# michelebanfi/qLDPC

Measured on AMD Instinct MI355X. Metric: syndromes/sec at 50 BP iters, [[288,12,18]] code, higher is better.
Workload: dtype f64; 1 GPU; BASELINE.json configs[3]: [[288,12,18]] BB code, sum-product BP, max_iter 50, every syndrome runs all 50 iterations (mode M2); max_iter=50, threads_per_block=1024, grid=512, lds_bytes=124000

## Files before the change

### qldpc_amd/csrc/qbp_kernels.hpp

```cpp
#pragma once

#include <hip/hip_runtime.h>
#include <stdint.h>

#include <type_traits>

#include "qbp_check.hpp"
#include "qbp_mc.hpp"

#ifndef QBP_WIDE_JG
#define QBP_WIDE_JG 4
#endif
#ifndef QBP_WIDE_HOLD_R
#define QBP_WIDE_HOLD_R 1
#endif
#ifndef QBP_WIDE_PACK
#define QBP_WIDE_PACK 0
#endif
#ifndef QBP_SMALL_HOLD_R
#define QBP_SMALL_HOLD_R 1
#endif
#ifndef QBP_SMALL_PACK
#define QBP_SMALL_PACK 0
#endif
#ifndef QBP_MC_HOLD_R
#define QBP_MC_HOLD_R 0
#endif
#ifndef QBP_MC_PACK
#define QBP_MC_PACK 0
#endif
#ifndef QBP_WORK_CHUNK_SMALL_CODES
#define QBP_WORK_CHUNK_SMALL_CODES 1
#endif
#ifndef QBP_WORK_CHUNK_FIXED
#define QBP_WORK_CHUNK_FIXED 0
#endif

namespace qbp {

constexpr int FUSED_R2_OFF_BYTES = 57344;

struct FusedParams {
    const uint8_t* syndromes;
    const double* prior;
    long long B;
    int m, n;
    int S;
    int slot_stride;
    int max_iter;
    unsigned flags;
    int padded;
    int n_words4;
    int r0_table;
    double alpha, damping, clip_llr;
    uint8_t* hard;
    uint8_t* converged;
    int32_t* iters;
    double* llr;
    const int32_t* tab_var;
    const uint16_t* tab_nbr;
    const uint32_t* tab_writer;
    const int32_t* iso_vars;
    int n_iso;
    unsigned long long* work_counter;
    const unsigned long long* lx_cols;
    long long trial_begin;
    unsigned long long seed;
    unsigned threshold;
    int draws;
    int half_distance;
    long long* counters;
    const uint8_t* errors_in;
    long long* fail_list;
    unsigned long long* fail_count;
    uint8_t* fail_syn;
    double* fail_llr;
    uint8_t* fail_hard;
    uint8_t* fail_err;
    const uint32_t* thr_cols;
    int n_budgets;
    int budgets[MAX_BUDGETS];
};

typedef const FusedParams __attribute__((address_space(4)))* ColdArgs;
__device__ __forceinline__ ColdArgs cold_args()
{
    ColdArgs p = (ColdArgs)__builtin_amdgcn_kernarg_segment_ptr();
    asm volatile("" : "+s"(p));
    return p;
}
#define COLD(field) (cold_args()->field)

__device__ __forceinline__ int work_chunk_for(int avg4)
{
    return avg4 < 12 ? 8 : avg4 < 28 ? 4 : avg4 < 60 ? 2 : 1;
}

__device__ __forceinline__ void mc_classify(unsigned long long* mc_lmask, int* mc_weight,
                                            int* mc_diff, int* cnt, int slot, int conv, int it,
                                            int half_distance, bool deferred)
{
    if (deferred) {
        cnt[0] += 1; cnt[6] += 1; cnt[7] += it;
        return;
    }
    const unsigned long long lm = mc_lmask[slot];
    const int ew = mc_weight[slot];
    const int df = mc_diff[slot];
    mc_lmask[slot] = 0ull; mc_weight[slot] = 0; mc_diff[slot] = 0;
    mc_count_trial(cnt, lm, ew, df, conv, it, half_distance);
}

template <int DC, int DV, int VARIANT, bool MC, bool FORCE_FULL, int MAX_THREADS, int MIN_WAVES_PER_SIMD,
          bool ONE_BARRIER = false>
__global__ __launch_bounds__(MAX_THREADS, MIN_WAVES_PER_SIMD) void bp_fused_kernel(const FusedParams P)
{
    constexpr bool ONE_BAR = ONE_BARRIER && FORCE_FULL && !MC;
    constexpr bool BUDGETS = MC && QBP_MC_BUDGETS != 0;
    extern __shared__ __attribute__((aligned(16))) double smem_all[];
    constexpr NpT np_tab = 0u;
    double* const smem = smem_all + NP_LDS_DOUBLES;
    const int tid = threadIdx.x;
    const int m = P.m;
    const int S = P.S;
    const int slot = tid / m;
    const int c = tid - slot * m;
    const bool lane_valid = slot < S;
    const bool leader = lane_valid && c == 0;
    const int sl = lane_valid ? slot : 0;

    double* const Rs = smem + (size_t)sl * P.slot_stride;
    const int zoff = DC * m;
    double* const pri_lds = smem + (ONE_BAR ? FUSED_R2_OFF_BYTES / 8 : 0) + (size_t)S * P.slot_stride;
    const bool use_r0 = !FORCE_FULL && P.r0_table != 0;
    double* const r0_lds = pri_lds + DC * m;
    long long* const next_work = reinterpret_cast<long long*>(r0_lds + (use_r0 ? 2 * DC * m : 0));
    long long* const chunk_ends = next_work + S;
    unsigned long long* const mc_lmask = reinterpret_cast<unsigned long long*>(chunk_ends + S);
    int* const words = reinterpret_cast<int*>(mc_lmask + S);
    int* const flag0 = words;
    int* const mc_weight = words + 3 * S;
    int* const mc_diff = words + 4 * S;
    int* const work_avg = words + 5 * S;
    int* const active_count = words + 6 * S;
    int slot_counters = NUM_COUNTERS;
    if constexpr (BUDGETS) slot_counters = 2 * COLD(n_budgets) * NUM_COUNTERS;
    int* const mc_count = words + 6 * S + 1 + sl * slot_counters;
    int* const var_lds = words + 6 * S + 1 + S * slot_counters;
    unsigned err_par = 0;
    auto err_buf = [&]() -> unsigned char* {
        const int n4 = COLD(n_words4) * 4;
        return reinterpret_cast<unsigned char*>(var_lds + DC * m) + (size_t)(sl + (err_par ? S : 0)) * n4;
    };

    auto check_step = [&](const double (&q)[DC], unsigned sb, auto&& put) {
        check_row<VARIANT, DC, (DC > 6)>(q, sb, P.alpha, true, np_tab, put);
    };

    constexpr bool PACK_NBR = (DC > 6 && QBP_WIDE_PACK != 0) || (MC && QBP_MC_PACK != 0) ||
                              (DC <= 6 && !MC && QBP_SMALL_PACK != 0);
    constexpr int NBR_W = PACK_NBR ? (DV + 1) / 2 : DV;
    unsigned nbr[DC][NBR_W];
    unsigned wmask = 0;
    unsigned vmask = 0;
#pragma unroll
    for (int j = 0; j < DC; ++j) {
        const int v = lane_valid ? P.tab_var[j * m + c] : -1;
        vmask |= (v >= 0 ? 1u : 0u) << j;
        if (slot == 0) {
            pri_lds[j * m + c] = v >= 0 ? P.prior[v] : __builtin_inf();
            var_lds[j * m + c] = v;
        }
#pragma unroll
        for (int k = 0; k < DV; ++k)
        {
            const unsigned o = lane_valid ? P.tab_nbr[(j * DV + k) * m + c] : (unsigned)zoff;
            if constexpr (PACK_NBR) {
                if (k & 1) nbr[j][k / 2] |= o << 16; else nbr[j][k / 2] = o;
            } else {
                nbr[j][k] = o;
            }
        }
    }
    if (lane_valid) wmask = P.tab_writer[c];
    if (lds_address(smem_all) != np_tab) __builtin_trap();
    np_tables_to_lds(smem_all, tid, blockDim.x);
    if (use_r0) __syncthreads();
    if (use_r0 && lane_valid && slot == 0) {
        double qp[DC];
#pragma unroll
        for (int j = 0; j < DC; ++j) qp[j] = pri_lds[j * m + c];
        check_step(qp, 0u, [&](int j, double r) { r0_lds[j * m + c] = r; });
        check_step(qp, 1u, [&](int j, double r) { r0_lds[(DC + j) * m + c] = r; });
    }

    const long long B = P.B;
    const long long total_slots = (long long)gridDim.x * S;
    const double one_minus_damping = 1.0 - P.damping;
    const int max_iter = P.max_iter;

    auto work_chunk = [&](long long handed_out, int by_cost) -> int {
        if (QBP_WORK_CHUNK_FIXED) return FORCE_FULL ? 1 : 8;
        const long long rem = B - handed_out;
        const int share = rem >= 16 * total_slots ? 8 : rem >= 8 * total_slots ? 4 : rem >= 4 * total_slots ? 2 : 1;
        const int ch = share > by_cost ? share : by_cost;
        const int f = QBP_WORK_CHUNK_SMALL_CODES ? (m <= 36 ? 4 : m <= 72 ? 2 : 1) : 1;
        return (f > 1 && ch == 8 && rem >= (long long)16 * f * total_slots) ? 8 * f : ch;
    };
    long long b = lane_valid ? (long long)blockIdx.x * S + slot : B;
    bool active = b < B;

    if (leader) {
        Rs[zoff] = 0.0;
        if constexpr (ONE_BAR) Rs[FUSED_R2_OFF_BYTES / 8 + zoff] = 0.0;
        flag0[slot] = 0;
        flag0[S + slot] = 0;
        flag0[2 * S + slot] = 0;
        mc_lmask[slot] = 0ull;
        mc_weight[slot] = 0;
        mc_diff[slot] = 0;
        if (slot == 0) *work_avg = 4 * P.max_iter;
        if constexpr (BUDGETS) {
            for (int i = 0; i < slot_counters; ++i) mc_count[i] = 0;
        } else if constexpr (MC) {
            for (int i = 0; i < NUM_COUNTERS; ++i) mc_count[i] = 0;
        }
        const int ch = work_chunk(9 * total_slots, 1);
        const long long first =
            B > total_slots ? total_slots + (long long)atomicAdd(P.work_counter, (unsigned long long)ch) : B;
        next_work[slot] = first;
        chunk_ends[slot] = first + ch;
    }
    if (tid == 0) {
        long long first = (long long)blockIdx.x * S;
        long long cnt = B - first;
        *active_count = (int)(cnt < 0 ? 0 : (cnt > S ? S : cnt));
    }

    constexpr bool HOLD_R = MC ? (QBP_MC_HOLD_R != 0 && DC <= 6) : (DC <= 6 ? QBP_SMALL_HOLD_R != 0 : QBP_WIDE_HOLD_R != 0);

    double Q[DC];
    double R[HOLD_R ? DC : 1];
    unsigned sbit = 0, ebits = 0;
    int it = 0;
    bool frozen = false;
    int bj = 0, ck_it = 0;

    auto start_syndrome = [&]() {
        it = 0;
        frozen = false;
        if constexpr (BUDGETS) { bj = 0; ck_it = COLD(budgets)[0] - 1; }
#pragma unroll
        for (int j = 0; j < DC; ++j) Q[j] = pri_lds[j * m + c];
        if constexpr (MC) {
            ebits = 0;
            const unsigned char* const err_lds = err_buf();
#pragma unroll
            for (int j = 0; j < DC; ++j) {
                const int v = var_lds[j * m + c];
                if (v >= 0) ebits |= (unsigned)err_lds[v] << j;
            }
            sbit = __builtin_popcount(ebits) & 1u;
        } else {
            sbit = COLD(syndromes)[b * m + c] & 1u;
        }
    };
    bool need_start = active;
    __syncthreads();

    int refill = 0;
    bool mc_pending = false;
    int mc_pending_conv = 0, mc_pending_it = 0;
    int mc_pending_row = 0;
    auto pending_row = [&]() -> int* {
        if constexpr (BUDGETS)
            return mc_count + ((mc_pending_conv ? COLD(n_budgets) : 0) + mc_pending_row) * NUM_COUNTERS;
        else
            return mc_count;
    };

    double val_keep[DC];
    auto emit_decode = [&](const double (&val)[DC], bool conv, int it_out) {
        const ColdArgs ca = cold_args();
        double* const o_llr = ca->llr;
        uint8_t* const o_hard = ca->hard;
        const long long row = b * ca->n;
#pragma unroll
        for (int j = 0; j < DC; ++j) {
            if ((wmask >> j) & 1u) {
                const long long o = row + var_lds[j * m + c];
                if (o_llr) o_llr[o] = val[j];
                if (o_hard) o_hard[o] = (uint8_t)(val[j] < 0.0);
            }
        }
        const int n_iso = ca->n_iso;
        for (int i = c; i < n_iso; i += m) {
            const int v = COLD(iso_vars)[i];
            const double pv = COLD(prior)[v];
            if (o_llr) o_llr[row + v] = pv;
            if (o_hard) o_hard[row + v] = pv < 0.0;
        }
        if (c == 0) {
            if (ca->converged) ca->converged[b] = conv;
            if (ca->iters) ca->iters[b] = it_out;
        }
    };
    int f_cur = 0, f_next = 1, f_prev = 2;
    int wg_it = 0;

    auto phase_body = [&](auto par_tag) -> bool {
        constexpr int PAR = decltype(par_tag)::value;
        double* const Rw = ONE_BAR ? Rs + PAR * (FUSED_R2_OFF_BYTES / 8) : Rs;
        double val_phase[DC];
        double (&val)[DC] = ONE_BAR ? val_keep : val_phase;
        if constexpr (MC) {
            if (need_start) {
                err_par ^= 1u;
                unsigned* const err_words = reinterpret_cast<unsigned*>(err_buf());
                const unsigned long long trial = (unsigned long long)(COLD(trial_begin) + b);
#if QBP_MC_COLS
                const uint32_t* const thr = COLD(thr_cols);
                for (int g = c; g < P.n_words4; g += m)
                    err_words[g] = mc_error_quad_cols(trial, g, COLD(draws), COLD(seed), thr);
#else
                const uint8_t* const ein = COLD(errors_in);
                for (int g = c; g < P.n_words4; g += m)
                    err_words[g] = ein ? mc_stored_quad(ein + b * COLD(n), g, COLD(n))
                                       : mc_error_quad(trial, g, COLD(draws), COLD(seed), COLD(threshold));
#endif
            }
            __syncthreads();
        }
        if (need_start) { start_syndrome(); need_start = false; }
        if (active) {
            if (use_r0 && it == 0) {
                const double* const r0 = r0_lds + (sbit ? DC * m : 0);
#pragma unroll
                for (int j = 0; j < DC; ++j) {
                    const double r = r0[j * m + c];
                    Rw[j * m + c] = r;
                    if constexpr (HOLD_R) R[j] = r;
                }
            } else {
                check_step(Q, sbit, [&](int j, double r) {
                    Rw[j * m + c] = r;
                    if constexpr (HOLD_R) R[j] = r;
                });
            }
        }
        __syncthreads();
        if (*active_count == 0) return true;

        if constexpr (ONE_BAR) {
            if (active && it > 0 && !frozen && flag0[f_prev * S + slot] == 0) {
                emit_decode(val, true, it - 1);
                frozen = true;
            }
        }
        if (active) {
            bool odd = sbit != 0;
            constexpr int JG = (DC * DV <= 18) ? DC : QBP_WIDE_JG;
#pragma unroll
            for (int j0 = 0; j0 < DC; j0 += JG) {
                double rr[JG][DV];
                double rown[HOLD_R ? 1 : JG];
#pragma unroll
                for (int jj = 0; jj < JG; ++jj) {
#pragma unroll
                    for (int k = 0; k < DV; ++k)
                        if (j0 + jj < DC) {
                            if constexpr (PACK_NBR) {
                                unsigned o;
                                unsigned pk = nbr[j0 + jj][k / 2];
                                asm volatile("" : "+v"(pk));
                                o = (k & 1) ? pk >> 16 : pk & 0xffffu;
                                rr[jj][k] = Rw[o];
                            } else {
                                rr[jj][k] = Rw[nbr[j0 + jj][k]];
                            }
                        }
                    if constexpr (!HOLD_R)
                        if (j0 + jj < DC) rown[jj] = Rw[(j0 + jj) * m + c];
                }
                __builtin_amdgcn_sched_barrier(0);
#pragma unroll
                for (int jj = 0; jj < JG; ++jj) {
                    const int j = j0 + jj;
                    if (j >= DC) break;
                    double s = rr[jj][0];
#pragma unroll
                    for (int k = 1; k < DV; ++k) s = s + rr[jj][k];
                    val[j] = s + pri_lds[j * m + c];
                    odd ^= val[j] < 0.0;
                    double r_own;
                    if constexpr (HOLD_R) r_own = R[j]; else r_own = rown[jj];
                    const double qn = val[j] - r_own;
                    if constexpr (VARIANT == 0) {
                        Q[j] = qn;
                    } else {
                        Q[j] = damped_q(qn, Q[j], P.damping, one_minus_damping, P.clip_llr);
                    }
                }
            }
            if (P.padded) {
#pragma unroll
                for (int j = 0; j < DC; ++j)
                    if (!((vmask >> j) & 1u)) Q[j] = __builtin_inf();
            }
            if (odd) flag0[f_cur * S + slot] = 1;
        }
        if (leader) {
            flag0[f_next * S + slot] = 0;
            if (refill) {
                long long nx = next_work[slot] + 1;
                if (nx == chunk_ends[slot]) {
                    const int ch = work_chunk(nx, refill);
                    nx = total_slots +
                         (long long)atomicAdd(COLD(work_counter), (unsigned long long)ch);
                    chunk_ends[slot] = nx + ch;
                }
                next_work[slot] = nx;
                refill = 0;
            }
            if constexpr (MC) {
                if (mc_pending) {
                    mc_classify(mc_lmask, mc_weight, mc_diff, pending_row(), slot, mc_pending_conv,
                                mc_pending_it, COLD(half_distance),
                                COLD(fail_list) != nullptr && !mc_pending_conv);
                    mc_pending = false;
                }
            }
        }
        const bool settle = !ONE_BAR || wg_it == max_iter - 1;
        if (settle) __syncthreads();

        if (active && settle) {
            const bool conv = flag0[f_cur * S + slot] == 0;
            const bool last = it == (ONE_BAR ? COLD(max_iter) : max_iter) - 1;
            bool emit_now = conv || last;
            if constexpr (BUDGETS) emit_now = conv || it == ck_it;
            if (!frozen && emit_now) {
                if constexpr (MC) {
                    const ColdArgs ca = cold_args();
                    long long rec = b;
                    if constexpr (BUDGETS) rec = (long long)bj * ca->B + b;
                    const long long row = rec * ca->n;
                    const int n_iso = ca->n_iso;
                    if (ca->fail_list != nullptr && !conv) {
                        double* const f_llr = ca->fail_llr;
                        uint8_t* const f_hard = ca->fail_hard;
                        uint8_t* const f_err = ca->fail_err;
                        ca->fail_syn[rec * m + c] = (uint8_t)sbit;
#pragma unroll
                        for (int j = 0; j < DC; ++j) {
                            if ((wmask >> j) & 1u) {
                                const long long o = row + var_lds[j * m + c];
                                f_llr[o] = val[j];
                                f_hard[o] = (uint8_t)(val[j] < 0.0);
                                f_err[o] = (uint8_t)((ebits >> j) & 1u);
                            }
                        }
                        const unsigned char* const err_lds = err_buf();
                        for (int i = c; i < n_iso; i += m) {
                            const int v = COLD(iso_vars)[i];
                            const double pv = COLD(prior)[v];
                            f_llr[row + v] = pv;
                            f_hard[row + v] = (uint8_t)(pv < 0.0);
                            f_err[row + v] = err_lds[v];
                        }
                        if constexpr (BUDGETS) {
                            if (c == 0) ca->fail_list[bj * ca->B + (long long)atomicAdd(ca->fail_count + bj, 1ull)] = b;
                        } else {
                            if (c == 0) ca->fail_list[atomicAdd(ca->fail_count, 1ull)] = b;
                        }
                    } else {
                    unsigned long long lm = 0ull;
                    int ew = 0;
                    unsigned df = 0;
                    const unsigned long long* const lx = ca->lx_cols;
#pragma unroll
                    for (int j = 0; j < DC; ++j) {
                        if ((wmask >> j) & 1u) {
                            const unsigned e = (ebits >> j) & 1u;
                            const unsigned res = (val[j] < 0.0 ? 1u : 0u) ^ e;
                            ew += (int)e;
                            df |= res;
                            const int v = var_lds[j * m + c];
                            if (res) lm ^= lx[v];
                        }
                    }
                    const unsigned char* const err_lds = err_buf();
                    for (int i = c; i < n_iso; i += m) {
                        const int v = COLD(iso_vars)[i];
                        const unsigned e = err_lds[v];
                        const unsigned res = (COLD(prior)[v] < 0.0 ? 1u : 0u) ^ e;
                        ew += (int)e;
                        df |= res;
                        if (res) lm ^= lx[v];
                    }
                    if (lm) atomicXor(&mc_lmask[slot], lm);
                    if (ew) atomicAdd(&mc_weight[slot], ew);
                    if (df) atomicOr(&mc_diff[slot], 1);
                    }
                    if (c == 0) {
                        mc_pending = true; mc_pending_conv = conv; mc_pending_it = it;
                        if constexpr (BUDGETS) mc_pending_row = bj;
                    }
                } else {
                    emit_decode(val, conv, it);
                }
            }
            if (conv) frozen = true;
            const bool finished = last || (conv && !FORCE_FULL);
            if (finished) {
                b = next_work[slot];
                if (b < B) {
                    need_start = true;
                    if (c == 0) {
                        if constexpr (FORCE_FULL) {
                            refill = 1;
                        } else {
                            const int a4 = *work_avg;
                            const int n4 = it * 4 > a4 ? it * 4 : a4 - (a4 >> 2) + it;
                            *work_avg = n4;
                            refill = work_chunk_for(n4);
                        }
                    }
                } else {
                    active = false;
                    if (c == 0) atomicSub(active_count, 1);
                }
            } else {
                if constexpr (BUDGETS) {
                    if (it == ck_it) { ++bj; ck_it = COLD(budgets)[bj] - 1; }
                }
                ++it;
            }
        } else if (active) {
            ++it;
        }
        {
            const int t = f_prev; f_prev = f_cur; f_cur = f_next; f_next = ONE_BAR ? t : f_prev;
            if constexpr (ONE_BAR) wg_it = wg_it == max_iter - 1 ? 0 : wg_it + 1;
        }
        return false;
    };
    for (;;) {
        if (phase_body(std::integral_constant<int, 0>{})) break;
        if constexpr (ONE_BAR) {
            if (phase_body(std::integral_constant<int, 1>{})) break;
        }
    }

    if constexpr (MC) {
        if (leader) {
            if (mc_pending)
                mc_classify(mc_lmask, mc_weight, mc_diff, pending_row(), slot, mc_pending_conv,
                            mc_pending_it, COLD(half_distance),
                            COLD(fail_list) != nullptr && !mc_pending_conv);
            if constexpr (!BUDGETS) {
                for (int i = 0; i < NUM_COUNTERS; ++i)
                    if (mc_count[i])
                        atomicAdd(reinterpret_cast<unsigned long long*>(COLD(counters) + i),
                                  (unsigned long long)mc_count[i]);
            }
        }
        if constexpr (BUDGETS) {
            __syncthreads();
            const int K = COLD(n_budgets);
            const int* const tab = words + 6 * S + 1;
            for (int t = tid; t < K * NUM_COUNTERS; t += blockDim.x) {
                const int j = t / NUM_COUNTERS, i = t - j * NUM_COUNTERS;
                long long sum = 0;
                for (int s = 0; s < S; ++s) {
                    const int* const rows = tab + s * slot_counters;
                    sum += rows[j * NUM_COUNTERS + i];
                    for (int jj = 0; jj <= j; ++jj) sum += rows[(K + jj) * NUM_COUNTERS + i];
                }
                if (sum)
                    atomicAdd(reinterpret_cast<unsigned long long*>(COLD(counters) + t), (unsigned long long)sum);
            }
        }
    }
}

#ifdef QBP_DEFINE_KERNELS
__global__ void debug_math_kernel(int kind, const double* x, double* y, long long n)
{
    __shared__ __attribute__((aligned(16))) double np_lds[NP_LDS_DOUBLES];
    np_tables_to_lds(np_lds, threadIdx.x, blockDim.x);
    const NpT np_tab = lds_address(np_lds);
    __syncthreads();
    const long long i = (long long)blockIdx.x * blockDim.x + threadIdx.x;
    if (i >= n) return;
    const double v = x[i];
    switch (kind) {
        case 0: y[i] = tanh_half_msg<0>(v, np_tab); break;
        case 1: y[i] = atanh2_msg(v, np_tab); break;
        case 4: y[i] = tanh_half(v); break;
        case 5: y[i] = atanh2(v); break;
        case 2: y[i] = __builtin_amdgcn_rcp(v); break;
        default: y[i] = div_nr(1.0, v); break;
    }
}

__global__ void mc_sample_kernel(uint8_t* errors, int n, long long T, long long trial_begin, int draws,
                                 unsigned long long seed, unsigned threshold)
{
    const int n4 = (n + 3) / 4;
    const long long i = (long long)blockIdx.x * blockDim.x + threadIdx.x;
    if (i >= T * n4) return;
    const long long b = i / n4;
    const int g = (int)(i - b * n4);
    const unsigned q = mc_error_quad((unsigned long long)(trial_begin + b), g, draws, seed, threshold);
#pragma unroll
    for (int k = 0; k < 4; ++k)
        if (4 * g + k < n) errors[b * n + 4 * g + k] = (uint8_t)((q >> (8 * k)) & 1u);
}

__global__ void mc_sample_cols_kernel(uint8_t* errors, int n, long long T, long long trial_begin, int draws,
                                      unsigned long long seed, const uint32_t* thr)
{
    const int n4 = (n + 3) / 4;
    const long long i = (long long)blockIdx.x * blockDim.x + threadIdx.x;
    if (i >= T * n4) return;
    const long long b = i / n4;
    const int g = (int)(i - b * n4);
    const unsigned q = mc_error_quad_cols((unsigned long long)(trial_begin + b), g, draws, seed, thr);
#pragma unroll
    for (int k = 0; k < 4; ++k)
        if (4 * g + k < n) errors[b * n + 4 * g + k] = (uint8_t)((q >> (8 * k)) & 1u);
}

#endif

}
```

Before: 6.615 million syndromes/s.

## Recompute early-converged decode values from stored R instead of keeping val registers

In the one-barrier path, the per-phase val_keep array that held decoded values across phases is removed. Early-convergence emission is now gated by a wave-wide check of the previous flags, and the posterior is recomputed from the other-parity R buffer in LDS plus the prior. Flags are initialised to 1 for inactive or frozen slots so the check rarely fires. This cuts register pressure and per-iteration emit checks, at the cost of a cold __syncthreads path and extra LDS reads when emission does happen.

```diff
diff --git a/qldpc_amd/csrc/qbp_kernels.hpp b/qldpc_amd/csrc/qbp_kernels.hpp
--- a/qldpc_amd/csrc/qbp_kernels.hpp
+++ b/qldpc_amd/csrc/qbp_kernels.hpp
@@ -183,6 +183,10 @@
         }
     }
     if (lane_valid) wmask = P.tab_writer[c];
+    auto nbr_at = [&](int j, int k) -> unsigned {
+        if constexpr (PACK_NBR) return (k & 1) ? nbr[j][k / 2] >> 16 : nbr[j][k / 2] & 0xffffu;
+        else return nbr[j][k];
+    };
     if (lds_address(smem_all) != np_tab) __builtin_trap();
     np_tables_to_lds(smem_all, tid, blockDim.x);
     if (use_r0) __syncthreads();
@@ -213,9 +217,7 @@
     if (leader) {
         Rs[zoff] = 0.0;
         if constexpr (ONE_BAR) Rs[FUSED_R2_OFF_BYTES / 8 + zoff] = 0.0;
-        flag0[slot] = 0;
-        flag0[S + slot] = 0;
-        flag0[2 * S + slot] = 0;
+        flag0[slot] = flag0[S + slot] = flag0[2 * S + slot] = (ONE_BAR && !active) ? 1 : 0;
         mc_lmask[slot] = 0ull;
         mc_weight[slot] = 0;
         mc_diff[slot] = 0;
@@ -243,7 +245,7 @@
     double R[HOLD_R ? DC : 1];
     unsigned sbit = 0, ebits = 0;
     int it = 0;
-    bool frozen = false;
+    bool frozen = ONE_BAR && !active;
     int bj = 0, ck_it = 0;
 
     auto start_syndrome = [&]() {
@@ -279,7 +281,6 @@
             return mc_count;
     };
 
-    double val_keep[DC];
     auto emit_decode = [&](const double (&val)[DC], bool conv, int it_out) {
         const ColdArgs ca = cold_args();
         double* const o_llr = ca->llr;
@@ -305,14 +306,41 @@
             if (ca->iters) ca->iters[b] = it_out;
         }
     };
+    auto emit_decode_1b = [&](auto&& val, bool conv, int it_out) {
+        const ColdArgs ca = cold_args();
+        double* const o_llr = ca->llr;
+        uint8_t* const o_hard = ca->hard;
+        const long long row = b * ca->n;
+        int ce = c;
+        asm volatile("" : "+v"(ce));
+#pragma unroll
+        for (int j = 0; j < DC; ++j) {
+            if ((wmask >> j) & 1u) {
+                const long long o = row + var_lds[j * m + ce];
+                const double v = val(j);
+                if (o_llr) o_llr[o] = v;
+                if (o_hard) o_hard[o] = (uint8_t)(v < 0.0);
+            }
+        }
+        const int n_iso = ca->n_iso;
+        for (int i = ce; i < n_iso; i += m) {
+            const int v = COLD(iso_vars)[i];
+            const double pv = COLD(prior)[v];
+            if (o_llr) o_llr[row + v] = pv;
+            if (o_hard) o_hard[row + v] = pv < 0.0;
+        }
+        if (ce == 0) {
+            if (ca->converged) ca->converged[b] = conv;
+            if (ca->iters) ca->iters[b] = it_out;
+        }
+    };
     int f_cur = 0, f_next = 1, f_prev = 2;
     int wg_it = 0;
 
     auto phase_body = [&](auto par_tag) -> bool {
         constexpr int PAR = decltype(par_tag)::value;
         double* const Rw = ONE_BAR ? Rs + PAR * (FUSED_R2_OFF_BYTES / 8) : Rs;
-        double val_phase[DC];
-        double (&val)[DC] = ONE_BAR ? val_keep : val_phase;
+        double val[DC];
         if constexpr (MC) {
             if (need_start) {
                 err_par ^= 1u;
@@ -331,7 +359,11 @@
             }
             __syncthreads();
         }
-        if (need_start) { start_syndrome(); need_start = false; }
+        if (need_start) {
+            start_syndrome();
+            if constexpr (ONE_BAR) if (c == 0) flag0[f_cur * S + slot] = 0;
+            need_start = false;
+        }
         if (active) {
             if (use_r0 && it == 0) {
                 const double* const r0 = r0_lds + (sbit ? DC * m : 0);
@@ -352,9 +384,34 @@
         if (*active_count == 0) return true;
 
         if constexpr (ONE_BAR) {
-            if (active && it > 0 && !frozen && flag0[f_prev * S + slot] == 0) {
-                emit_decode(val, true, it - 1);
-                frozen = true;
+            bool wg_emit = false;
+            if (wg_it > 0) {
+                const int* const fp = flag0 + f_prev * S;
+                const int sp = tid & 63;
+                wg_emit = QBP_WAVE_ANY(fp[sp < S ? sp : S - 1] == 0);
+                if (S > 64) {
+                    QBP_COLD_BEGIN();
+                    for (int s0 = 64; s0 < S; s0 += 64)
+                        wg_emit |= QBP_WAVE_ANY(fp[s0 + sp < S ? s0 + sp : S - 1] == 0);
+                    QBP_COLD_END();
+                }
+            }
+            if (wg_emit) {
+                QBP_COLD_BEGIN();
+                if (active && !frozen && flag0[f_prev * S + slot] == 0) {
+                    const double* const Rp = Rs + (PAR ^ 1) * (FUSED_R2_OFF_BYTES / 8);
+                    emit_decode_1b([&](int j) {
+                        __builtin_amdgcn_sched_barrier(0);
+                        double s = Rp[nbr_at(j, 0)];
+#pragma unroll
+                        for (int k = 1; k < DV; ++k) s = s + Rp[nbr_at(j, k)];
+                        return s + pri_lds[j * m + c];
+                    }, true, it - 1);
+                    frozen = true;
+                    if (c == 0) flag0[f_cur * S + slot] = 1;
+                }
+                __syncthreads();
+                QBP_COLD_END();
             }
         }
         if (active) {
@@ -410,7 +467,7 @@
             if (odd) flag0[f_cur * S + slot] = 1;
         }
         if (leader) {
-            flag0[f_next * S + slot] = 0;
+            flag0[f_next * S + slot] = (ONE_BAR && frozen) ? 1 : 0;
             if (refill) {
                 long long nx = next_work[slot] + 1;
                 if (nx == chunk_ends[slot]) {
@@ -507,7 +564,8 @@
                         if constexpr (BUDGETS) mc_pending_row = bj;
                     }
                 } else {
-                    emit_decode(val, conv, it);
+                    if constexpr (ONE_BAR) emit_decode_1b([&](int j) { return val[j]; }, conv, it);
+                    else emit_decode(val, conv, it);
                 }
             }
             if (conv) frozen = true;
@@ -528,6 +586,7 @@
                     }
                 } else {
                     active = false;
+                    if constexpr (ONE_BAR) frozen = true;
                     if (c == 0) atomicSub(active_count, 1);
                 }
             } else {
```

Result: slower. 6.547 million syndromes/s (-1.0%).
